# GANtastic3/MaskCycleGAN-VC

Measured on AMD Instinct MI355X. Metric: train iters/s (full G+D step), 80x64 mel bs=1, higher is better.
Workload: dtype f32

## Files before the change

include/mcvc.h:

```cpp
#ifndef MCVC_H
#define MCVC_H

#ifdef __cplusplus
extern "C" {
#endif

#define MCVC_ABI_VERSION 3
#define MCVC_GEN_NPARAMS 110
#define MCVC_DISC_NPARAMS 20
#define MCVC_N_MEL 80

int mcvc_version(void);

int mcvc_set_deterministic(int on);
int mcvc_get_deterministic(void);
int mcvc_set_precise(int on);
int mcvc_get_precise(void);
int mcvc_set_trunk_persistent(int on);

int mcvc_twin_begin(void);
int mcvc_twin_switch(void);
int mcvc_twin_end(void);
int mcvc_twin_launches(void);

long long mcvc_gen_packed_floats(void);
long long mcvc_disc_packed_floats(void);
long long mcvc_gen_stash_floats(int B, int T);
long long mcvc_gen_scratch_floats(int B, int T);
long long mcvc_disc_stash_floats(int B, int T);
// ... 151 lines not shown
int mcvc_instnorm_act_backward(const float* x, const float* gamma, const float* beta, const float* gamma_gate,
                               const float* beta_gate, const float* stats, float* dy, float* dx,
                               float* dgamma, float* dbeta, float* dgamma_gate, float* dbeta_gate,
                               int N, int C, int H, int W, int act, void* stream);

int mcvc_trunk_layer_forward(const float* x, const float* w, const float* bias, const float* gamma, const float* beta, const float* w_gate,
                             const float* bias_gate, const float* gamma_gate, const float* beta_gate, const float* residual, float* conv_out,
                             float* stats, float* y, int B, int Cin, int T4, int Cout, int KW, void* stream);

int mcvc_batched_gemm(const float* a, const float* b, float* c, int nbatch, int M, int N, int K, int lda, int ldb, int ldc,
                      long long a_stride, long long b_stride, long long c_stride, void* stream);

int mcvc_bias_grad(const float* dy, float* db, int N, int C, int P, void* stream);
int mcvc_act_forward(float* x, float* y, int N, int C, int P, int act, void* stream);
int mcvc_act_backward(const float* x, float* dy, float* dx, int N, int C, int P, int act, void* stream);
int mcvc_fif_input(const float* x, const float* mask, float* xin, int N, int P, void* stream);
int mcvc_fif_input_grad(const float* dxin, const float* mask, float* dx, int N, int P, int accumulate, void* stream);

int mcvc_trace_enable(int on);
int mcvc_trace_kinds(void);
const char* mcvc_trace_kind_name(int kind);
int mcvc_trace_collect(double* out);
int mcvc_trace_collect_raw(double* out, int max_records);

#ifdef __cplusplus
}
#endif
#endif
```

maskcyclegan-vc_amd/csrc/fewout_kernels.hip:

```cpp
#include "mcvc_common.h"
#include "trace.h"
#include "launch.h"
#include <stdlib.h>

namespace {

constexpr int kFewTW = 64;
constexpr int kFewTH = 16;
constexpr int kFewCC = 4;

__device__ __attribute__((aligned(16))) float g_few_zero[64];

__device__ __forceinline__ void glds4(const float* g, float* l)
{
    __builtin_amdgcn_global_load_lds((const __attribute__((address_space(1))) void*)g,
                                     (__attribute__((address_space(3))) void*)l, 4, 0, 0);
}

struct FewArgs {
    const float* x; const float* w; const float* bias;
    float* y; float* y_slabs;
    long long x_sb, x_sc, y_sb, y_sc, slab_stride;
    int x_sh, y_sh, y_sw;
    int Cin, H, W, Cout, OH, OW, KH, pad_h, pad_w;
// ... 537 lines not shown
            }
        }
    }
    __syncthreads();
    if (rg < ngr) red[rg * ntap + tap] = acc;
    __syncthreads();
    if (tid < ntap && (int)blockIdx.y < units) {
        float s = 0.f;
        for (int g = 0; g < ngr; ++g) s += red[g * ntap + tid];
        float* d = a.dw + (long long)ci * ntap + tid;
        if (gridDim.y > 1) unsafeAtomicAdd(d, s); else *d += s;
    }
}

constexpr int kCin1Band = 20;
struct WgradCin1KArgs { const float* x; long long x_sn; int x_sh; const float* dy; long long dy_sn; long long dy_sc; int dy_sh; float* dw; int NB; int H; int W; };
__global__ void __launch_bounds__(256) wgrad_cin1_kernel(const Twin<WgradCin1KArgs> tw)
{
    const WgradCin1KArgs ka_ = tw.v[blockIdx.z];
    const float* __restrict__ x = ka_.x;
    long long x_sn = ka_.x_sn;
    int x_sh = ka_.x_sh;
    const float* __restrict__ dy = ka_.dy;
    long long dy_sn = ka_.dy_sn;
    long long dy_sc = ka_.dy_sc;
    int dy_sh = ka_.dy_sh;
    float* __restrict__ dw = ka_.dw;
    int NB = ka_.NB;
    int H = ka_.H;
    int W = ka_.W;
    extern __shared__ float sm[];
    const int XW = W + 2;
    float* xs = sm;
    float* red = sm + (kCin1Band + 2) * XW;
    const int tid = threadIdx.x, co = blockIdx.x;
    const int bands = (H + kCin1Band - 1) / kCin1Band;
    const int units = NB * bands;
    float acc[9];
#pragma unroll
    for (int t = 0; t < 9; ++t) acc[t] = 0.f;
    for (int u = blockIdx.y; u < units; u += gridDim.y) {
        const int n = u / bands, h0 = (u - n * bands) * kCin1Band;
        const int rows = (H - h0 < kCin1Band) ? H - h0 : kCin1Band;
        const float* xp = x + (long long)n * x_sn;
        __syncthreads();
        for (int i = tid; i < (rows + 2) * XW; i += 256) {
            const int r = i / XW, c = i - r * XW;
            const int ih = h0 + r - 1, iw = c - 1;
            xs[i] = (ih >= 0 && ih < H && iw >= 0 && iw < W) ? xp[(long long)ih * x_sh + iw] : 0.f;
        }
        __syncthreads();
        const float* dp = dy + (long long)n * dy_sn + (long long)co * dy_sc + (long long)h0 * dy_sh;
        for (int i = tid; i < rows * W; i += 256) {
            const int r = i / W, c = i - r * W;
            const float d = dp[(long long)r * dy_sh + c];
            const float* xr = xs + r * XW + c;
#pragma unroll
            for (int kh = 0; kh < 3; ++kh)
#pragma unroll
                for (int kw = 0; kw < 3; ++kw) acc[kh * 3 + kw] = fmaf(d, xr[kh * XW + kw], acc[kh * 3 + kw]);
        }
    }
#pragma unroll
    for (int t = 0; t < 9; ++t) {
#pragma unroll
        for (int o = 32; o > 0; o >>= 1) acc[t] += __shfl_xor(acc[t], o, 64);
    }
    __syncthreads();
    if ((tid & 63) == 0) {
#pragma unroll
        for (int t = 0; t < 9; ++t) red[(tid >> 6) * 9 + t] = acc[t];
    }
    __syncthreads();
    if (tid < 9 && (int)blockIdx.y < units) {
        const float v = (red[tid] + red[9 + tid]) + (red[18 + tid] + red[27 + tid]);
        float* d = dw + co * 9 + tid;
        if (gridDim.y > 1) unsafeAtomicAdd(d, v); else *d += v;
    }
}

}

namespace {

constexpr int kW1Ch = 16, kW1PW = 84;
template <int BAND> constexpr int kW1PlaneOf = (BAND + 4) * kW1PW + 4;
constexpr int kW1DyW = 64 + 32;
struct W1Args {
    const float* x; long long x_sn, x_sc; int x_sh;
    const float* dy; long long dy_sn; int dy_sh;
    float* dw;
// ... 91 lines not shown
    }
}

}

namespace {

constexpr int kW2Co = 64;
template <int BAND> constexpr int kW2DyPitch = BAND * 64 + 4;
constexpr int kW2XP = 84;
struct W2Args {
    const float* x; long long x_sn, x_sc; int x_sh;
    const float* dy; long long dy_sn, dy_sc; int dy_sh;
    float* dw;
    int N, Cin, Cout, H, W, bands, units, atomic;
};
template <int CI, int kW2Band>
__global__ void __launch_bounds__(256, 2) wgrad_cin2_mfma_kernel(const Twin<W2Args> tw)
{
    constexpr int kW2DyP = kW2DyPitch<kW2Band>;
    const W2Args a = tw.v[blockIdx.z];
    extern __shared__ __attribute__((aligned(16))) float sm[];
    float* dys = sm;
    float* xs = sm + kW2Co * kW2DyP;
    const int tid = threadIdx.x, lane = tid & 63;
    const int wave = __builtin_amdgcn_readfirstlane(tid >> 6);
    const int ln = lane & 15, kq = lane >> 4;
    const int co0 = blockIdx.x * kW2Co;
    typedef float f32x4w __attribute__((ext_vector_type(4)));
    f32x4w acc[CI][5];
#pragma unroll
    for (int ci = 0; ci < CI; ++ci)
#pragma unroll
        for (int kh = 0; kh < 5; ++kh) acc[ci][kh] = f32x4w{0.f, 0.f, 0.f, 0.f};
    constexpr int P4 = kW2XP / 4, XR = kW2Band + 4;
    for (int u = blockIdx.y; u < a.units; u += gridDim.y) {
        const int n = u / a.bands, h0 = (u - n * a.bands) * kW2Band;
        __syncthreads();
        {
            constexpr int NIT = kW2Co * kW2Band * 16 / 256;
            float4 v[NIT];
#pragma unroll
            for (int it = 0; it < NIT; ++it) {
                const int i = tid + it * 256;
                const int co = i / (kW2Band * 16), rem = i - co * (kW2Band * 16);
                const int r = rem >> 4, c4 = rem & 15;
                v[it] = make_float4(0.f, 0.f, 0.f, 0.f);
                if (co0 + co < a.Cout && h0 + r < a.H)
                    v[it] = *reinterpret_cast<const float4*>(a.dy + (long long)n * a.dy_sn + (long long)(co0 + co) * a.dy_sc + (long long)(h0 + r) * a.dy_sh + 4 * c4);
            }
#pragma unroll
            for (int it = 0; it < NIT; ++it) {
                const int i = tid + it * 256;
// ... 42 lines not shown
    __syncthreads();
    float* red = sm;
    const int per = a.Cin * 75;
#pragma unroll
    for (int ci = 0; ci < CI; ++ci) {
        if (ci >= a.Cin) break;
#pragma unroll
        for (int kh = 0; kh < 5; ++kh)
#pragma unroll
            for (int q = 0; q < 4; ++q) {
                const int kw = 4 * kq + q;
                if (kw < 15) red[(wave * 16 + ln) * per + (ci * 5 + kh) * 15 + kw] = acc[ci][kh][q];
            }
    }
    __syncthreads();
    int nco = a.Cout - co0; if (nco > kW2Co) nco = kW2Co;
    float* d0 = a.dw + (long long)co0 * per;
    for (int i = tid; i < nco * per; i += 256) {
        if (a.atomic) unsafeAtomicAdd(d0 + i, red[i]); else d0[i] += red[i];
    }
}

}

bool mcvc_wgrad_cin2_applies(const ConvProblem& p, const WgradIO& io)
{
    static const int en = mcvc_knob("MCVC_WGRAD_CIN2_MFMA", 1);
    return en && p.Cin >= 1 && p.Cin <= 2 && p.KH == 5 && p.KW == 15 && p.stride == 1 && p.pad_h == 2 && p.pad_w == 7 && p.W == 64 && p.OH == p.H &&
           p.OW == p.W && (io.x_sh & 3) == 0 && (io.x_sc & 3) == 0 && (io.x_sb & 3) == 0 && (io.dy_sh & 3) == 0 && (io.dy_sc & 3) == 0 &&
           (io.dy_sb & 3) == 0 && ((reinterpret_cast<unsigned long long>(io.x) | reinterpret_cast<unsigned long long>(io.dy)) & 15ull) == 0;
}

int mcvc_wgrad_cin2_launch(const ConvProblem& p, int NB, const WgradIO& io, float* dw, hipStream_t s)
{
// ... 2 lines not shown
    w.x = io.x; w.x_sn = io.x_sb; w.x_sc = io.x_sc; w.x_sh = io.x_sh;
    w.dy = io.dy; w.dy_sn = io.dy_sb; w.dy_sc = io.dy_sc; w.dy_sh = io.dy_sh; w.dw = dw;
    const int blocks = cdiv_i(p.Cout, kW2Co);
    const int band = ((long long)blocks * NB * cdiv_i(p.H, 4) < 256) ? 2 : 4;
    w.N = NB; w.Cin = p.Cin; w.Cout = p.Cout; w.H = p.H; w.W = p.W; w.bands = cdiv_i(p.H, band); w.units = NB * w.bands;
    int nch = 1;
    static const int wgs = mcvc_knob("MCVC_WGRAD_CIN2_WGS", 512);
    if (!mcvc_deterministic())
        while (2 * nch <= w.units && blocks * nch < wgs) nch *= 2;
    w.atomic = nch > 1 ? 1 : 0;
    size_t lds = (size_t)(kW2Co * (band * 64 + 4) + 2 * (band + 4) * kW2XP) * sizeof(float);
    const size_t lds_out = (size_t)kW2Co * p.Cin * 75 * sizeof(float);
    if (lds < lds_out) lds = lds_out;
    TraceScope ts(K_WGRAD_4x1, s, 2.0 * NB * p.H * p.W * p.Cout * p.Cin * p.KH * p.KW, 4.0 * ((double)NB * p.Cout * p.H * p.W + (double)NB * p.Cin * p.H * p.W));
    const dim3 grid((unsigned)blocks, (unsigned)nch);
    if (p.Cin == 1) { if (band == 2) mcvc_launch((wgrad_cin2_mfma_kernel<1, 2>), grid, dim3(256), lds, s, w); else mcvc_launch((wgrad_cin2_mfma_kernel<1, 4>), grid, dim3(256), lds, s, w); }
    else { if (band == 2) mcvc_launch((wgrad_cin2_mfma_kernel<2, 2>), grid, dim3(256), lds, s, w); else mcvc_launch((wgrad_cin2_mfma_kernel<2, 4>), grid, dim3(256), lds, s, w); }
    return (int)hipGetLastError();
}

bool mcvc_wgrad_cout1_applies(const ConvProblem& p)
{
    if (p.Cout != 1 || p.stride != 1 || p.KH * p.KW > 128 || p.OH != p.H || p.OW != p.W) return false;
    const int XW = p.W + p.KW - 1;
    const size_t lds = ((size_t)(p.H + p.KH - 1) * XW + (size_t)p.H * p.W + 256) * sizeof(float);
    return lds <= 64 * 1024;
}

int mcvc_wgrad_cout1_launch(const ConvProblem& p, int NB, const WgradIO& io, float* dw, hipStream_t s)
{
    if (!mcvc_wgrad_cout1_applies(p)) return MCVC_ERR_INVALID;
    FewWgradArgs a{};
// ... 34 lines not shown

bool mcvc_wgrad_cin1_applies(const ConvProblem& p)
{
    return p.Cin == 1 && p.KH == 3 && p.KW == 3 && p.stride == 1 && p.pad_h == 1 && p.pad_w == 1 && p.OH == p.H && p.OW == p.W && p.W <= 512;
}

int mcvc_wgrad_cin1_launch(const ConvProblem& p, int NB, const WgradIO& io, float* dw, hipStream_t s)
{
    if (!mcvc_wgrad_cin1_applies(p)) return MCVC_ERR_INVALID;
    const int units = NB * cdiv_i(p.H, kCin1Band);
    int nchunk = 1;
    if (!mcvc_deterministic())
        while (2 * nchunk <= units && p.Cout * nchunk < 1024) nchunk *= 2;
    const size_t lds = ((size_t)(kCin1Band + 2) * (p.W + 2) + 36) * sizeof(float);
    TraceScope ts(K_WGRAD_SMALLK, s, 2.0 * NB * p.H * p.W * p.Cout * 9, 4.0 * ((double)NB * p.Cout * p.H * p.W + (double)NB * p.H * p.W));
    mcvc_launch(wgrad_cin1_kernel, dim3((unsigned)p.Cout, (unsigned)nchunk), dim3(256), lds, s, WgradCin1KArgs{io.x, io.x_sb, io.x_sh, io.dy, io.dy_sb, io.dy_sc, io.dy_sh, dw, NB, p.H, p.W});
    return (int)hipGetLastError();
}
```

maskcyclegan-vc_amd/csrc/mcvc_common.h:

```cpp
#pragma once
#include <hip/hip_runtime.h>
#include <stdint.h>
#include <stddef.h>

typedef float f32x16 __attribute__((ext_vector_type(16)));
typedef float f32x4 __attribute__((ext_vector_type(4)));

#define MCVC_OK 0
#define MCVC_ERR_INVALID 1001
#define MCVC_ERR_WORKSPACE 1002

int mcvc_deterministic();

#ifdef MCVC_EXPERIMENTS
#include <cstdlib>
static inline int mcvc_knob(const char* name, int dflt) { const char* e = getenv(name); return e ? atoi(e) : dflt; }
static inline bool mcvc_knob_set(const char* name) { return getenv(name) != nullptr; }
#else
static inline int mcvc_knob(const char*, int dflt) { return dflt; }
static inline bool mcvc_knob_set(const char*) { return false; }
#endif

static inline int cdiv_i(int a, int b) { return (a + b - 1) / b; }
static inline long long cdiv_ll(long long a, long long b) { return (a + b - 1) / b; }
// ... 141 lines not shown
int mcvc_disc_out_fwd_launch(const float* x, const float* w, const float* bias, float* logit, float* out, int NB, int C, int H, int W, hipStream_t s);
int mcvc_disc_conv1_fwd_launch(const float* x, const float* w, const float* bias, float* c0, float* y0, int NB, int Cout, int H, int W, hipStream_t s, int xs = 0);
int mcvc_disc_out_dgrad_launch(const float* dlogit, const float* w, float* dx, int NB, int C, int H, int W, hipStream_t s);

struct WgradIO {
    const float* x; long long x_sb, x_sc; int x_sh;
    const float* dy; long long dy_sb, dy_sc; int dy_sh;
};
int mcvc_wgrad_launch(const ConvProblem& p, int NB, const WgradIO& io, float* dw, float* slabs, long long slab_cap_floats, hipStream_t s);
bool mcvc_wgrad_cin2_applies(const ConvProblem& p, const WgradIO& io);
int mcvc_wgrad_cin2_launch(const ConvProblem& p, int NB, const WgradIO& io, float* dw, hipStream_t s);
bool mcvc_wgrad_cout1_applies(const ConvProblem& p);
bool mcvc_wgrad_cin1_applies(const ConvProblem& p);
int mcvc_wgrad_cin1_launch(const ConvProblem& p, int NB, const WgradIO& io, float* dw, hipStream_t s);
int mcvc_wgrad_cout1_launch(const ConvProblem& p, int NB, const WgradIO& io, float* dw, hipStream_t s);
long long mcvc_wgrad_plan_slab_floats(const ConvProblem& p, int NB);

struct SmallKJob { const float* x; const float* dy; float* dw; int Cin, Cout; int xB; };
#define MCVC_SMALLK_MAX_JOBS 24
int mcvc_wgrad_smallk_batch_launch(const SmallKJob* jobs, int njobs, int B, int T4, hipStream_t s);
bool mcvc_wgrad_smallk_batch_applies(int B, int T4);

int mcvc_norm_fwd_launch(const NormArgs& a, hipStream_t s);
int mcvc_norm_bwd_launch(const NormBwdArgs& a, hipStream_t s);
int mcvc_act_fwd_launch(const ActArgs& a, hipStream_t s);
int mcvc_act_bwd_launch(const ActBwdArgs& a, hipStream_t s);
```

maskcyclegan-vc_amd/csrc/net.hip:

```cpp
#include "mcvc_common.h"
#include "twin.h"
#include "pack.h"
#include "misc.h"
#include "trunk.h"
#include "wino.h"
#include "wino4.h"
#include "sgemm.h"
#include "sampler.h"
#include "audio.h"
#include "vocoder.h"
#include "griffinlim.h"
#include "../../include/mcvc.h"
#include <string.h>
#include <algorithm>
#include <map>
#include <mutex>
#include <vector>

static int g_deterministic = [] { const char* e = getenv("MCVC_DETERMINISTIC"); return (e && atoi(e) != 0) ? 1 : 0; }();
int mcvc_deterministic() { return g_deterministic; }

namespace {

constexpr float kInEps = 1e-5f;

struct View { float* p; long long sb, sc; int sh; };
struct CView { const float* p; long long sb, sc; int sh; };
static inline CView cv(const View& v) { return CView{v.p, v.sb, v.sc, v.sh}; }

struct Exec {
    hipStream_t s;
    bool dry;
    int err;
    bool fine_ms = false;
    float* slabs;
// ... 1619 lines not shown
        CView dyv{GB, 512LL * 20 * W4, 20LL * W4, W4};
        conv_wgrad(ex, g.ds2, G, B, 40, W2, CView{st + o.y2, 256LL * 40 * W2, 40LL * W2, W2}, dyv);
        conv_dgrad(ex, g.ds2, packed, B, 40, W2, dyv, View{GA, 256LL * 40 * W2, 40LL * W2, W2}, (long long)B * 256 * 40 * W2, 0, 1, &ns);
    }
    if (milestones && ex.fine_ms) record_milestone(ex, milestones[2]);
    GB = nextGB();
    norm_bwd(ex, st + o.c2, 512LL * 40 * W2, 40LL * W2, normp(P, G, 6, 7, 10, 11), st + o.s2, GA, 256LL * 40 * W2, 40LL * W2, W2,
             (long long)B * 256 * 40 * W2, ns, GB, 512LL * 40 * W2, 40LL * W2, W2, 0, B, 256, 40, W2, ACT_GLU);
    {
        CView dyv{GB, 512LL * 40 * W2, 40LL * W2, W2};
        conv_wgrad(ex, g.ds1, G, B, 80, T, CView{st + o.y1, 128LL * 80 * T, 80LL * T, T}, dyv);
        conv_dgrad(ex, g.ds1, packed, B, 80, T, dyv, View{GA, 128LL * 80 * T, 80LL * T, T}, (long long)B * 128 * 80 * T, 0, 1, &ns);
    }
    if (milestones && ex.fine_ms) record_milestone(ex, milestones[3]);
    GB = nextGB();
    act_bwd(ex, st + o.c1, GA, (long long)B * 128 * 80 * T, ns, GB, B, 128, 80 * T, ACT_GLU);
    {
        CView dyv{GB, 256LL * 80 * T, 80LL * T, T};
        ex.br1_on_main = (dx == nullptr) ? 1 : 0;
        conv_wgrad(ex, g.conv1, G, B, 80, T, CView{st + o.xin, 2LL * 80 * T, 80LL * T, T}, dyv);
        ex.br1_on_main = 0;
        conv_bias_grad(ex, g.conv1, G, B, dyv, 80 * T);
        if (dx) {
            conv_dgrad(ex, g.conv1, packed, B, 80, T, dyv, View{GA, 2LL * 80 * T, 80LL * T, T}, (long long)B * 2 * 80 * T, 0, 1, &ns);
            if (!ex.dry) ex.fail(mcvc_mask_grad_launch(GA, ex.slabs, (long long)B * 2 * 80 * T, ns, mask, dx, B, 80 * T, 2, accumulate_dx, ex.s));
        }
    }
    if (ex.no_join) ex.readers.clear(); else join_aux(ex);
}

struct DiscNet { ConvSpec conv1, ds[3], outc; long long packed_floats; };
static DiscNet build_disc()
{
    DiscNet n{};
    long long cur = 0;
    n.conv1 = mk(1, 128, 1, 3, 3, 1, 1, 1, 0, 1, -1, -1, 1);
    n.ds[0] = mk(128, 256, 1, 3, 3, 2, 1, 1, 2, 3, -1, -1, 0);
// ... 147 lines not shown
                     GB, (long long)Co * pl, pl, pitch, 0, B, Co, Ho, Wo, ACT_SILU);
            ex.wgrad_x_xs = 1;
            conv_wgrad(ex, n.ds[i], G, B, Hi, Wi, CView{hin, (long long)Ci * 4 * xpl, 4 * xpl, Wi}, CView{GB, (long long)Co * pl, pl, pitch});
            ex.wgrad_x_xs = 0;
            conv_dgrad_igemm(ex, n.ds[i], packed, B, Hi, Wi, GB, View{GA, (long long)Ci * Hi * Wi, (long long)Hi * Wi, Wi}, (long long)B * Ci * Hi * Wi, 0, 1, &ns);
            continue;
        }
        norm_bwd(ex, st + o.c[i], (long long)Co * Ho * Wo, (long long)Ho * Wo, normp(P, G, 4 + 4 * i, 5 + 4 * i), st + o.s[i],
                 GA, (long long)Co * Ho * Wo, (long long)Ho * Wo, Wo, (long long)B * Co * Ho * Wo, ns,
                 GB, (long long)Co * Ho * Wo, (long long)Ho * Wo, Wo, 0, B, Co, Ho, Wo, ACT_SILU);
        CView dyv{GB, (long long)Co * Ho * Wo, (long long)Ho * Wo, Wo};
        conv_wgrad(ex, n.ds[i], G, B, Hi, Wi, CView{hin, (long long)Ci * Hi * Wi, (long long)Hi * Wi, Wi}, dyv);
        conv_dgrad(ex, n.ds[i], packed, B, Hi, Wi, dyv, View{GA, (long long)Ci * Hi * Wi, (long long)Hi * Wi, Wi}, (long long)B * Ci * Hi * Wi, 0, 1, &ns);
    }
    GB = nextGB();
    act_bwd(ex, st + o.c0, GA, (long long)B * 128 * 80 * T, ns, GB, B, 128, 80 * T, ACT_SILU);
    {
        CView dyv{GB, 128LL * 80 * T, 80LL * T, T};
        conv_wgrad(ex, n.conv1, G, B, 80, T, CView{st + o.total, 80LL * T, 80LL * T, T}, dyv);
        conv_bias_grad(ex, n.conv1, G, B, dyv, 80 * T);
        if (dx) {
            conv_dgrad(ex, n.conv1, packed, B, 80, T, dyv, View{GA, 80LL * T, 80LL * T, T}, (long long)B * 80 * T, 0, 1, &ns);
            if (!ex.dry) ex.fail(mcvc_mask_grad_launch(GA, ex.slabs, (long long)B * 80 * T, ns, nullptr, dx, B, 80 * T, 1, accumulate_dx, ex.s));
        }
    }
    join_aux(ex);
}

struct Needs { long long slab, wslab, sg, sgw; };

template <class F>
static Needs cached_needs(int kind, int B, int T, F&& dry_run)
// ... 73 lines not shown
int mcvc_twin_end(void)
{
    if (!g_mcvc_twin) return MCVC_ERR_INVALID;
    TwinCtx* t = g_mcvc_twin;
    g_mcvc_twin = nullptr;
    const int phase = t->phase;
    t->phase = 0;
    if (t->err) return t->err;
    if (phase != 2 || t->next != t->recs.size()) return MCVC_ERR_INVALID;
    return 0;
}
int mcvc_twin_launches(void) { return (int)t_twin_ctx.recs.size(); }

int mcvc_set_deterministic(int on) { const int was = g_deterministic; g_deterministic = on ? 1 : 0; return was; }
int mcvc_get_deterministic(void) { return g_deterministic; }
int mcvc_set_precise(int on) { const int was = g_precise; g_precise = on ? 1 : 0; return was; }
int mcvc_get_precise(void) { return g_precise; }
int mcvc_set_trunk_persistent(int on) { const int was = g_trunk_net; g_trunk_net = (on == 2) ? 2 : (on ? 1 : 0); return was; }

long long mcvc_gen_packed_floats(void) { return gen_net().packed_floats; }
long long mcvc_disc_packed_floats(void) { return disc_net().packed_floats; }
int mcvc_gen_out_frames(int T) { return gen_dims(1, T).Wu2; }
int mcvc_disc_out_frames(int T) { return disc_dims(1, T).W[3]; }

long long mcvc_gen_stash_floats(int B, int T) { return gen_stash(gen_dims(B, T)).total; }

long long mcvc_gen_scratch_floats(int B, int T)
{
    const Needs nd = gen_needs(B, T);
    return gen_scratch(gen_dims(B, T)).slabs + nd.slab + nd.sg + nd.sgw + nd.wslab + 64;
// ... 805 lines not shown

int mcvc_act_forward(float* x, float* y, int N, int C, int P, int act, void* stream)
{
    Exec ex{}; ex.s = (hipStream_t)stream;
    act_fwd(ex, x, 0, 1, y, N, C, P, act);
    return ex.err;
}

int mcvc_act_backward(const float* x, float* dy, float* dx, int N, int C, int P, int act, void* stream)
{
    Exec ex{}; ex.s = (hipStream_t)stream;
    act_bwd(ex, x, dy, 0, 1, dx, N, C, P, act);
    return ex.err;
}

int mcvc_fif_input(const float* x, const float* mask, float* xin, int N, int P, void* stream)
{
    return mcvc_prep_input_launch(x, mask, xin, N, P, (hipStream_t)stream);
}

int mcvc_fif_input_grad(const float* dxin, const float* mask, float* dx, int N, int P, int accumulate, void* stream)
{
    return mcvc_mask_grad_launch(dxin, nullptr, 0, 1, mask, dx, N, P, 2, accumulate, (hipStream_t)stream);
}

}
```

maskcyclegan-vc_amd/mask_cyclegan_vc/_hip.py:

```python
from __future__ import annotations

import ctypes
import os
from ctypes import c_float, c_int, c_longlong, c_void_p

import torch

_HERE = os.path.dirname(os.path.abspath(__file__))
LIB_PATH = os.environ.get("MCVC_LIB") or os.path.join(os.path.dirname(_HERE), "lib", "libmcvc_hip.so")

ABI_VERSION = 3
GEN_NPARAMS = 110
DISC_NPARAMS = 20
N_MEL = 80

_lib = None

_PP = ctypes.POINTER(c_void_p)

_SIGS = {
    "mcvc_version": (c_int, []),
    "mcvc_set_deterministic": (c_int, [c_int]),
    "mcvc_get_deterministic": (c_int, []),
    "mcvc_set_precise": (c_int, [c_int]),
    "mcvc_get_precise": (c_int, []),
    "mcvc_set_trunk_persistent": (c_int, [c_int]),
    "mcvc_twin_begin": (c_int, []),
    "mcvc_twin_switch": (c_int, []),
    "mcvc_twin_end": (c_int, []),
    "mcvc_twin_launches": (c_int, []),
    "mcvc_gen_packed_floats": (c_longlong, []),
    "mcvc_disc_packed_floats": (c_longlong, []),
    "mcvc_gen_stash_floats": (c_longlong, [c_int, c_int]),
    "mcvc_gen_scratch_floats": (c_longlong, [c_int, c_int]),
    "mcvc_disc_stash_floats": (c_longlong, [c_int, c_int]),
    "mcvc_disc_scratch_floats": (c_longlong, [c_int, c_int]),
    "mcvc_gen_out_frames": (c_int, [c_int]),
    "mcvc_disc_out_frames": (c_int, [c_int]),
# ... 73 lines not shown
    "mcvc_conv2d_dgrad": (c_int, [c_void_p] * 5 + [c_int] * 11 + [c_void_p]),
    "mcvc_conv2d_wgrad_slab_floats": (c_longlong, [c_int] * 10),
    "mcvc_conv2d_wgrad": (c_int, [c_void_p] * 4 + [c_longlong] + [c_int] * 10 + [c_void_p]),
    "mcvc_layer_packed_floats": (c_longlong, [c_int] * 8),
    "mcvc_layer_scratch_floats": (c_longlong, [c_int] * 11),
    "mcvc_layer_pack": (c_int, [c_void_p] * 5 + [c_int] * 8 + [c_void_p]),
    "mcvc_layer_forward": (c_int, [c_void_p] * 6 + [c_longlong] + [c_int] * 13 + [c_void_p]),
    "mcvc_layer_dgrad": (c_int, [c_void_p] * 6 + [c_longlong] + [c_int] * 12 + [c_void_p]),
    "mcvc_layer_wgrad": (c_int, [c_void_p] * 5 + [c_longlong] + [c_int] * 12 + [c_void_p]),
    "mcvc_trunk_layer_backward": (c_int, [c_void_p] * 19 + [c_int] * 5 + [c_void_p]),
    "mcvc_instnorm_act_forward": (c_int, [c_void_p] * 8 + [c_int] * 5 + [c_void_p]),
    "mcvc_instnorm_act_backward": (c_int, [c_void_p] * 12 + [c_int] * 5 + [c_void_p]),
    "mcvc_trunk_layer_forward": (c_int, [c_void_p] * 13 + [c_int] * 5 + [c_void_p]),
    "mcvc_batched_gemm": (c_int, [c_void_p] * 3 + [c_int] * 7 + [c_longlong] * 3 + [c_void_p]),
    "mcvc_bias_grad": (c_int, [c_void_p, c_void_p, c_int, c_int, c_int, c_void_p]),
    "mcvc_act_forward": (c_int, [c_void_p, c_void_p, c_int, c_int, c_int, c_int, c_void_p]),
    "mcvc_act_backward": (c_int, [c_void_p, c_void_p, c_void_p, c_int, c_int, c_int, c_int, c_void_p]),
    "mcvc_fif_input": (c_int, [c_void_p, c_void_p, c_void_p, c_int, c_int, c_void_p]),
    "mcvc_fif_input_grad": (c_int, [c_void_p, c_void_p, c_void_p, c_int, c_int, c_int, c_void_p]),
    "mcvc_trace_enable": (c_int, [c_int]),
    "mcvc_trace_kinds": (c_int, []),
    "mcvc_trace_kind_name": (ctypes.c_char_p, [c_int]),
    "mcvc_trace_collect": (c_int, [ctypes.POINTER(ctypes.c_double)]),
    "mcvc_trace_collect_raw": (c_int, [ctypes.POINTER(ctypes.c_double), c_int]),
}

EXPORTED_SYMBOLS = tuple(_SIGS)


def lib():
# ... 63 lines not shown
```

Baseline: 177.9.

## Fuse activation backward and bias grad into first-layer weight-gradient kernels

Folds the GLU backward (generator conv1) and SiLU backward (discriminator conv1) into the weight-gradient kernels. Each kernel now sums the split-K gradient slabs, applies the activation derivative, and accumulates the bias gradient while staging dy. This removes separate act_bwd and bias_grad launches and the round trip of the intermediate dy through memory. When dx is needed the generator path can still write dy_out or run the plain wgrad on a side stream. In exchange the wgrad kernels carry more loads and sigmoid math, and the stream and event handling gets more complex.

After: 179.3, median of 3. About the same (+0.8%).

```diff
diff --git a/include/mcvc.h b/include/mcvc.h
--- a/include/mcvc.h
+++ b/include/mcvc.h
@@ -13,6 +13,7 @@
 int mcvc_version(void);
 
 int mcvc_set_deterministic(int on);
+int mcvc_set_first_layer_fusion(int mode);
 int mcvc_get_deterministic(void);
 int mcvc_set_precise(int on);
 int mcvc_get_precise(void);
@@ -194,6 +195,10 @@
 int mcvc_bias_grad(const float* dy, float* db, int N, int C, int P, void* stream);
 int mcvc_act_forward(float* x, float* y, int N, int C, int P, int act, void* stream);
 int mcvc_act_backward(const float* x, float* dy, float* dx, int N, int C, int P, int act, void* stream);
+int mcvc_gen_conv1_backward(const float* xin, const float* g, const float* g_slabs, int nslab, const float* c1, float* dy_out, float* dw,
+                            float* dw_gate, float* db, float* db_gate, int N, int C, int H, int W, void* stream);
+int mcvc_disc_conv1_backward(const float* x, const float* g, const float* g_slabs, int nslab, const float* c0, float* dw, float* db,
+                             int N, int C, int H, int W, void* stream);
 int mcvc_fif_input(const float* x, const float* mask, float* xin, int N, int P, void* stream);
 int mcvc_fif_input_grad(const float* dxin, const float* mask, float* dx, int N, int P, int accumulate, void* stream);
 
diff --git a/maskcyclegan-vc_amd/csrc/fewout_kernels.hip b/maskcyclegan-vc_amd/csrc/fewout_kernels.hip
--- a/maskcyclegan-vc_amd/csrc/fewout_kernels.hip
+++ b/maskcyclegan-vc_amd/csrc/fewout_kernels.hip
@@ -575,7 +575,12 @@
 }
 
 constexpr int kCin1Band = 20;
-struct WgradCin1KArgs { const float* x; long long x_sn; int x_sh; const float* dy; long long dy_sn; long long dy_sc; int dy_sh; float* dw; int NB; int H; int W; };
+__device__ __forceinline__ float fl_sigmoid(float v) { return 1.0f / (1.0f + expf(-v)); }
+struct WgradCin1KArgs {
+    const float* x; long long x_sn; int x_sh; const float* dy; long long dy_sn; long long dy_sc; int dy_sh; float* dw; int NB; int H; int W;
+    const float* slabs; long long slab_stride; int nslab; const float* c0; long long c_sn; float* db;
+};
+template <bool ACT>
 __global__ void __launch_bounds__(256) wgrad_cin1_kernel(const Twin<WgradCin1KArgs> tw)
 {
     const WgradCin1KArgs ka_ = tw.v[blockIdx.z];
@@ -595,6 +600,7 @@
     float* xs = sm;
     float* red = sm + (kCin1Band + 2) * XW;
     const int tid = threadIdx.x, co = blockIdx.x;
+    float bsum = 0.f;
     const int bands = (H + kCin1Band - 1) / kCin1Band;
     const int units = NB * bands;
     float acc[9];
@@ -614,7 +620,21 @@
         const float* dp = dy + (long long)n * dy_sn + (long long)co * dy_sc + (long long)h0 * dy_sh;
         for (int i = tid; i < rows * W; i += 256) {
             const int r = i / W, c = i - r * W;
-            const float d = dp[(long long)r * dy_sh + c];
+            float d = dp[(long long)r * dy_sh + c];
+            if (ACT) {
+                const long long go = (long long)n * dy_sn + (long long)co * dy_sc + (long long)(h0 + r) * dy_sh + c;
+                for (int sl = 1; sl < ka_.nslab; sl += 4) {
+                    float u[4];
+#pragma unroll
+                    for (int k = 0; k < 4; ++k) { const int s_ = (sl + k < ka_.nslab) ? sl + k : ka_.nslab - 1; u[k] = ka_.slabs[(long long)(s_ - 1) * ka_.slab_stride + go]; }
+#pragma unroll
+                    for (int k = 0; k < 4; ++k) if (sl + k < ka_.nslab) d += u[k];
+                }
+                const float x0 = ka_.c0[(long long)n * ka_.c_sn + (long long)co * dy_sc + (long long)(h0 + r) * dy_sh + c];
+                const float sg = fl_sigmoid(x0);
+                d = d * (sg * (1.0f + x0 * (1.0f - sg)));
+                bsum += d;
+            }
             const float* xr = xs + r * XW + c;
 #pragma unroll
             for (int kh = 0; kh < 3; ++kh)
@@ -626,16 +646,26 @@
     for (int t = 0; t < 9; ++t) {
 #pragma unroll
         for (int o = 32; o > 0; o >>= 1) acc[t] += __shfl_xor(acc[t], o, 64);
+    }
+    if (ACT) {
+#pragma unroll
+        for (int o = 32; o > 0; o >>= 1) bsum += __shfl_xor(bsum, o, 64);
     }
     __syncthreads();
     if ((tid & 63) == 0) {
 #pragma unroll
         for (int t = 0; t < 9; ++t) red[(tid >> 6) * 9 + t] = acc[t];
+        if (ACT) red[36 + (tid >> 6)] = bsum;
     }
     __syncthreads();
     if (tid < 9 && (int)blockIdx.y < units) {
         const float v = (red[tid] + red[9 + tid]) + (red[18 + tid] + red[27 + tid]);
         float* d = dw + co * 9 + tid;
+        if (gridDim.y > 1) unsafeAtomicAdd(d, v); else *d += v;
+    }
+    if (ACT && tid == 9 && (int)blockIdx.y < units && ka_.db) {
+        const float v = (red[36] + red[37]) + (red[38] + red[39]);
+        float* d = ka_.db + co;
         if (gridDim.y > 1) unsafeAtomicAdd(d, v); else *d += v;
     }
 }
@@ -757,8 +787,23 @@
     const float* dy; long long dy_sn, dy_sc; int dy_sh;
     float* dw;
     int N, Cin, Cout, H, W, bands, units, atomic;
+    const float* g; const float* slabs; long long slab_stride; int nslab; const float* c; long long c_sn;
+    float* dy_out; float* dw1; float* db[2];
 };
-template <int CI, int kW2Band>
+__device__ __forceinline__ float4 w2_ld4(const float* p) { return *reinterpret_cast<const float4*>(p); }
+__device__ __forceinline__ float4 w2_add4(const float4& a, const float4& b) { return make_float4(a.x + b.x, a.y + b.y, a.z + b.z, a.w + b.w); }
+__device__ __forceinline__ float4 w2_slab_sum4(float4 t, const float* slabs, long long stride, long long off, int nslab)
+{
+    for (int sl = 1; sl < nslab; sl += 4) {
+        float4 u[4];
+#pragma unroll
+        for (int k = 0; k < 4; ++k) { const int s_ = (sl + k < nslab) ? sl + k : nslab - 1; u[k] = w2_ld4(slabs + (long long)(s_ - 1) * stride + off); }
+#pragma unroll
+        for (int k = 0; k < 4; ++k) if (sl + k < nslab) t = w2_add4(t, u[k]);
+    }
+    return t;
+}
+template <int CI, int kW2Band, bool GLU>
 __global__ void __launch_bounds__(256, 2) wgrad_cin2_mfma_kernel(const Twin<W2Args> tw)
 {
     constexpr int kW2DyP = kW2DyPitch<kW2Band>;
@@ -777,9 +822,76 @@
 #pragma unroll
         for (int kh = 0; kh < 5; ++kh) acc[ci][kh] = f32x4w{0.f, 0.f, 0.f, 0.f};
     constexpr int P4 = kW2XP / 4, XR = kW2Band + 4;
+    constexpr int kStageIt = kW2Co * kW2Band * 16 / 256;
+    const int br = (GLU && co0 >= a.Cout) ? 1 : 0;
+    const int cb0 = co0 - br * a.Cout;
+    float bacc[GLU ? kStageIt : 1];
+#pragma unroll
+    for (int it = 0; it < (GLU ? kStageIt : 1); ++it) bacc[it] = 0.f;
     for (int u = blockIdx.y; u < a.units; u += gridDim.y) {
         const int n = u / a.bands, h0 = (u - n * a.bands) * kW2Band;
         __syncthreads();
+        if constexpr (GLU) {
+            constexpr int LPC = kW2Band * 16, CS = 256 / LPC;
+            constexpr int CH = kW2Band == 2 ? 4 : 2;
+            const int co_t = tid / LPC, r = (tid % LPC) >> 4, c4 = tid & 15;
+            const long long P = (long long)a.H * 64;
+            const bool ok = h0 + r < a.H;
+            const long long po = (long long)(h0 + r) * 64 + 4 * c4;
+            const long long go = ((long long)n * a.Cout + cb0 + co_t) * P + po;
+            const float* cp = a.c + (long long)n * a.c_sn + (long long)(cb0 + co_t) * P + po;
+            const float* dp = a.dy + (long long)n * a.dy_sn + (long long)(co0 + co_t) * a.dy_sc + (long long)(h0 + r) * a.dy_sh + 4 * c4;
+            float* op = a.dy_out + ((long long)n * 2 * a.Cout + co0 + co_t) * P + po;
+            float* lp = dys + co_t * kW2DyP + r * 64 + 4 * c4;
+#pragma unroll
+            for (int base = 0; base < kStageIt; base += CH) {
+                float4 gv[CH], vv[CH], tv[CH], sv[CH][4];
+#pragma unroll
+                for (int k = 0; k < CH; ++k) {
+                    const long long cs = (long long)(base + k) * CS;
+                    gv[k] = vv[k] = tv[k] = make_float4(0.f, 0.f, 0.f, 0.f);
+                    if (ok) {
+                        if (a.g) {
+                            gv[k] = w2_ld4(a.g + go + cs * P);
+                            vv[k] = w2_ld4(cp + cs * P); tv[k] = w2_ld4(cp + (cs + a.Cout) * P);
+                            if (a.nslab > 1) {
+#pragma unroll
+                                for (int q = 0; q < 4; ++q) {
+                                    const int s_ = (1 + q < a.nslab) ? 1 + q : a.nslab - 1;
+                                    sv[k][q] = w2_ld4(a.slabs + (long long)(s_ - 1) * a.slab_stride + go + cs * P);
+                                }
+                            }
+                        } else {
+                            gv[k] = w2_ld4(dp + cs * a.dy_sc);
+                        }
+                    }
+                }
+#pragma unroll
+                for (int k = 0; k < CH; ++k) {
+                    const long long cs = (long long)(base + k) * CS;
+                    float4 d = gv[k];
+                    if (a.g && ok) {
+                        if (a.nslab > 1) {
+#pragma unroll
+                            for (int q = 0; q < 4; ++q) if (1 + q < a.nslab) d = w2_add4(d, sv[k][q]);
+                            if (a.nslab > 5) d = w2_slab_sum4(d, a.slabs + 4 * a.slab_stride, a.slab_stride, go + cs * P, a.nslab - 4);
+                        }
+                        const float dv[4] = {d.x, d.y, d.z, d.w}, xv[4] = {vv[k].x, vv[k].y, vv[k].z, vv[k].w}, tg[4] = {tv[k].x, tv[k].y, tv[k].z, tv[k].w};
+                        float o[4];
+#pragma unroll
+                        for (int e = 0; e < 4; ++e) {
+                            const float sg = fl_sigmoid(tg[e]);
+                            o[e] = br ? dv[e] * xv[e] * sg * (1.0f - sg) : dv[e] * sg;
+                        }
+                        d = make_float4(o[0], o[1], o[2], o[3]);
+                        if (a.dy_out) *reinterpret_cast<float4*>(op + cs * P) = d;
+                    }
+                    *reinterpret_cast<float4*>(lp + (base + k) * CS * kW2DyP) = d;
+                    bacc[base + k] += (d.x + d.y) + (d.z + d.w);
+                }
+                __builtin_amdgcn_sched_barrier(0);
+            }
+        } else
         {
             constexpr int NIT = kW2Co * kW2Band * 16 / 256;
             float4 v[NIT];
@@ -852,10 +964,24 @@
             }
     }
     __syncthreads();
-    int nco = a.Cout - co0; if (nco > kW2Co) nco = kW2Co;
-    float* d0 = a.dw + (long long)co0 * per;
+    int nco = a.Cout - cb0; if (nco > kW2Co) nco = kW2Co;
+    float* d0 = (br ? a.dw1 : a.dw) + (long long)cb0 * per;
     for (int i = tid; i < nco * per; i += 256) {
         if (a.atomic) unsafeAtomicAdd(d0 + i, red[i]); else d0[i] += red[i];
+    }
+    if constexpr (GLU) {
+        constexpr int LPC = kW2Band * 16;
+        float* db = a.db[br];
+#pragma unroll
+        for (int it = 0; it < kStageIt; ++it) {
+            float v = bacc[it];
+#pragma unroll
+            for (int o = LPC / 2; o > 0; o >>= 1) v += __shfl_xor(v, o, 64);
+            if (db && (tid & (LPC - 1)) == 0) {
+                float* d = db + cb0 + (tid + it * 256) / LPC;
+                if (a.atomic) unsafeAtomicAdd(d, v); else *d += v;
+            }
+        }
     }
 }
 
@@ -888,8 +1014,40 @@
     if (lds < lds_out) lds = lds_out;
     TraceScope ts(K_WGRAD_4x1, s, 2.0 * NB * p.H * p.W * p.Cout * p.Cin * p.KH * p.KW, 4.0 * ((double)NB * p.Cout * p.H * p.W + (double)NB * p.Cin * p.H * p.W));
     const dim3 grid((unsigned)blocks, (unsigned)nch);
-    if (p.Cin == 1) { if (band == 2) mcvc_launch((wgrad_cin2_mfma_kernel<1, 2>), grid, dim3(256), lds, s, w); else mcvc_launch((wgrad_cin2_mfma_kernel<1, 4>), grid, dim3(256), lds, s, w); }
-    else { if (band == 2) mcvc_launch((wgrad_cin2_mfma_kernel<2, 2>), grid, dim3(256), lds, s, w); else mcvc_launch((wgrad_cin2_mfma_kernel<2, 4>), grid, dim3(256), lds, s, w); }
+    if (p.Cin == 1) { if (band == 2) mcvc_launch((wgrad_cin2_mfma_kernel<1, 2, false>), grid, dim3(256), lds, s, w); else mcvc_launch((wgrad_cin2_mfma_kernel<1, 4, false>), grid, dim3(256), lds, s, w); }
+    else { if (band == 2) mcvc_launch((wgrad_cin2_mfma_kernel<2, 2, false>), grid, dim3(256), lds, s, w); else mcvc_launch((wgrad_cin2_mfma_kernel<2, 4, false>), grid, dim3(256), lds, s, w); }
+    return (int)hipGetLastError();
+}
+
+int mcvc_wgrad_cin2_glu_launch(const ConvProblem& p, int NB, const WgradIO& io, const ActGradSrc* g, float* dy_out, float* dw0, float* dw1,
+                               float* db0, float* db1, hipStream_t s)
+{
+    if (!mcvc_wgrad_cin2_applies(p, io) || (p.Cout % kW2Co) != 0 || !dw0 || !dw1) return MCVC_ERR_INVALID;
+    W2Args w{};
+    w.x = io.x; w.x_sn = io.x_sb; w.x_sc = io.x_sc; w.x_sh = io.x_sh;
+    w.dy = io.dy; w.dy_sn = io.dy_sb; w.dy_sc = io.dy_sc; w.dy_sh = io.dy_sh; w.dw = dw0; w.dw1 = dw1; w.db[0] = db0; w.db[1] = db1;
+    if (g) {
+        if (!g->g || !g->c || g->nslab < 1 || (g->nslab > 1 && (!g->slabs || (g->slab_stride & 3))) || (g->c_sb & 3)) return MCVC_ERR_INVALID;
+        if ((reinterpret_cast<unsigned long long>(g->g) | reinterpret_cast<unsigned long long>(g->c) | reinterpret_cast<unsigned long long>(g->slabs) |
+             reinterpret_cast<unsigned long long>(dy_out)) & 15ull) return MCVC_ERR_INVALID;
+        w.g = g->g; w.slabs = g->slabs; w.slab_stride = g->slab_stride; w.nslab = g->nslab; w.c = g->c; w.c_sn = g->c_sb; w.dy_out = dy_out;
+    } else if (!io.dy) return MCVC_ERR_INVALID;
+    const int blocks = p.Cout / kW2Co;
+    const int band = ((long long)blocks * NB * cdiv_i(p.H, 4) < 256) ? 2 : 4;
+    w.N = NB; w.Cin = p.Cin; w.Cout = p.Cout; w.H = p.H; w.W = p.W; w.bands = cdiv_i(p.H, band); w.units = NB * w.bands;
+    int nch = 1;
+    static const int wgs = mcvc_knob("MCVC_WGRAD_CIN2_WGS", 512);
+    if (!mcvc_deterministic())
+        while (2 * nch <= w.units && blocks * nch < wgs) nch *= 2;
+    w.atomic = nch > 1 ? 1 : 0;
+    size_t lds = (size_t)(kW2Co * (band * 64 + 4) + 2 * (band + 4) * kW2XP) * sizeof(float);
+    const size_t lds_out = (size_t)kW2Co * p.Cin * 75 * sizeof(float);
+    if (lds < lds_out) lds = lds_out;
+    TraceScope ts(K_WGRAD_4x1, s, 2.0 * NB * p.H * p.W * 2 * p.Cout * p.Cin * p.KH * p.KW,
+                  4.0 * ((double)NB * 2 * p.Cout * p.H * p.W * (g ? 1.0 + 0.5 * g->nslab + (dy_out ? 1 : 0) : 1.0) + (double)NB * p.Cin * p.H * p.W));
+    const dim3 grid((unsigned)(2 * blocks), (unsigned)nch);
+    if (band == 2) mcvc_launch((wgrad_cin2_mfma_kernel<2, 2, true>), grid, dim3(256), lds, s, w);
+    else mcvc_launch((wgrad_cin2_mfma_kernel<2, 4, true>), grid, dim3(256), lds, s, w);
     return (int)hipGetLastError();
 }
 
@@ -954,6 +1112,22 @@
         while (2 * nchunk <= units && p.Cout * nchunk < 1024) nchunk *= 2;
     const size_t lds = ((size_t)(kCin1Band + 2) * (p.W + 2) + 36) * sizeof(float);
     TraceScope ts(K_WGRAD_SMALLK, s, 2.0 * NB * p.H * p.W * p.Cout * 9, 4.0 * ((double)NB * p.Cout * p.H * p.W + (double)NB * p.H * p.W));
-    mcvc_launch(wgrad_cin1_kernel, dim3((unsigned)p.Cout, (unsigned)nchunk), dim3(256), lds, s, WgradCin1KArgs{io.x, io.x_sb, io.x_sh, io.dy, io.dy_sb, io.dy_sc, io.dy_sh, dw, NB, p.H, p.W});
+    mcvc_launch(wgrad_cin1_kernel<false>, dim3((unsigned)p.Cout, (unsigned)nchunk), dim3(256), lds, s,
+                WgradCin1KArgs{io.x, io.x_sb, io.x_sh, io.dy, io.dy_sb, io.dy_sc, io.dy_sh, dw, NB, p.H, p.W, nullptr, 0, 1, nullptr, 0, nullptr});
     return (int)hipGetLastError();
 }
+
+int mcvc_wgrad_cin1_silu_launch(const ConvProblem& p, int NB, const float* x, long long x_sb, int x_sh, const ActGradSrc& g, float* dw, float* db, hipStream_t s)
+{
+    if (!mcvc_wgrad_cin1_applies(p) || !x || !g.g || !g.c || !dw || g.nslab < 1 || (g.nslab > 1 && !g.slabs)) return MCVC_ERR_INVALID;
+    const int units = NB * cdiv_i(p.H, kCin1Band);
+    int nchunk = 1;
+    if (!mcvc_deterministic())
+        while (2 * nchunk <= units && p.Cout * nchunk < 1024) nchunk *= 2;
+    const size_t lds = ((size_t)(kCin1Band + 2) * (p.W + 2) + 40) * sizeof(float);
+    const long long P = (long long)p.H * p.W;
+    TraceScope ts(K_WGRAD_SMALLK, s, 2.0 * NB * p.H * p.W * p.Cout * 10, 4.0 * ((double)(g.nslab + 1) * NB * p.Cout * p.H * p.W + (double)NB * p.H * p.W));
+    mcvc_launch(wgrad_cin1_kernel<true>, dim3((unsigned)p.Cout, (unsigned)nchunk), dim3(256), lds, s,
+                WgradCin1KArgs{x, x_sb, x_sh, g.g, (long long)p.Cout * P, P, p.W, dw, NB, p.H, p.W, g.slabs, g.slab_stride, g.nslab, g.c, g.c_sb, db});
+    return (int)hipGetLastError();
+}
diff --git a/maskcyclegan-vc_amd/csrc/mcvc_common.h b/maskcyclegan-vc_amd/csrc/mcvc_common.h
--- a/maskcyclegan-vc_amd/csrc/mcvc_common.h
+++ b/maskcyclegan-vc_amd/csrc/mcvc_common.h
@@ -179,6 +179,10 @@
 bool mcvc_wgrad_cin1_applies(const ConvProblem& p);
 int mcvc_wgrad_cin1_launch(const ConvProblem& p, int NB, const WgradIO& io, float* dw, hipStream_t s);
 int mcvc_wgrad_cout1_launch(const ConvProblem& p, int NB, const WgradIO& io, float* dw, hipStream_t s);
+struct ActGradSrc { const float* g; const float* slabs; long long slab_stride; int nslab; const float* c; long long c_sb; };
+int mcvc_wgrad_cin2_glu_launch(const ConvProblem& p, int NB, const WgradIO& io, const ActGradSrc* g, float* dy_out, float* dw0, float* dw1,
+                               float* db0, float* db1, hipStream_t s);
+int mcvc_wgrad_cin1_silu_launch(const ConvProblem& p, int NB, const float* x, long long x_sb, int x_sh, const ActGradSrc& g, float* dw, float* db, hipStream_t s);
 long long mcvc_wgrad_plan_slab_floats(const ConvProblem& p, int NB);
 
 struct SmallKJob { const float* x; const float* dy; float* dw; int Cin, Cout; int xB; };
diff --git a/maskcyclegan-vc_amd/csrc/net.hip b/maskcyclegan-vc_amd/csrc/net.hip
--- a/maskcyclegan-vc_amd/csrc/net.hip
+++ b/maskcyclegan-vc_amd/csrc/net.hip
@@ -19,6 +19,7 @@
 
 static int g_deterministic = [] { const char* e = getenv("MCVC_DETERMINISTIC"); return (e && atoi(e) != 0) ? 1 : 0; }();
 int mcvc_deterministic() { return g_deterministic; }
+static int g_first_layer = mcvc_knob("MCVC_FIRST_LAYER_FUSION", 1);
 
 namespace {
 
@@ -1668,13 +1669,39 @@
     }
     if (milestones && ex.fine_ms) record_milestone(ex, milestones[3]);
     GB = nextGB();
-    act_bwd(ex, st + o.c1, GA, (long long)B * 128 * 80 * T, ns, GB, B, 128, 80 * T, ACT_GLU);
+    const ConvProblem p1{2, 80, T, 128, 80, T, 5, 15, 1, 2, 7};
+    const WgradIO io1{st + o.xin, 2LL * 80 * T, 80LL * T, T, GB, 256LL * 80 * T, 80LL * T, T};
+    const bool fuse1 = g_first_layer && !ex.dry && G && G[g.conv1.wi[0]] && G[g.conv1.wi[1]] && mcvc_wgrad_cin2_applies(p1, io1);
+    const bool form1 = fuse1 && (dx == nullptr || g_first_layer == 2);
+    if (!form1) act_bwd(ex, st + o.c1, GA, (long long)B * 128 * 80 * T, ns, GB, B, 128, 80 * T, ACT_GLU);
     {
         CView dyv{GB, 256LL * 80 * T, 80LL * T, T};
-        ex.br1_on_main = (dx == nullptr) ? 1 : 0;
-        conv_wgrad(ex, g.conv1, G, B, 80, T, CView{st + o.xin, 2LL * 80 * T, 80LL * T, T}, dyv);
-        ex.br1_on_main = 0;
-        conv_bias_grad(ex, g.conv1, G, B, dyv, 80 * T);
+        float* const db0 = (fuse1 && g.conv1.has_bias_grad) ? G[g.conv1.bi[0]] : nullptr;
+        float* const db1 = (fuse1 && g.conv1.has_bias_grad) ? G[g.conv1.bi[1]] : nullptr;
+        if (form1) {
+            const ActGradSrc src{GA, ex.slabs, (long long)B * 128 * 80 * T, ns, st + o.c1, 256LL * 80 * T};
+            if (dx) wait_readers(ex, GB);
+            ex.fail(mcvc_wgrad_cin2_glu_launch(p1, B, io1, &src, dx ? GB : nullptr, G[g.conv1.wi[0]], G[g.conv1.wi[1]], db0, db1, ex.s));
+        } else if (fuse1) {
+            hipStream_t ws = ex.s;
+            if (ex.s2) {
+                hipEvent_t e = pool_event();
+                ex.fail(mcvc_event_record(e, ex.s));
+                ex.fail(mcvc_stream_wait(ex.s2, e));
+                ws = ex.s2;
+            }
+            ex.fail(mcvc_wgrad_cin2_glu_launch(p1, B, io1, nullptr, nullptr, G[g.conv1.wi[0]], G[g.conv1.wi[1]], db0, db1, ws));
+            if (ex.s2) {
+                hipEvent_t e = pool_event();
+                ex.fail(mcvc_event_record(e, ex.s2));
+                ex.readers.emplace_back((const void*)GB, e);
+            }
+        } else {
+            ex.br1_on_main = (dx == nullptr) ? 1 : 0;
+            conv_wgrad(ex, g.conv1, G, B, 80, T, CView{st + o.xin, 2LL * 80 * T, 80LL * T, T}, dyv);
+            ex.br1_on_main = 0;
+            conv_bias_grad(ex, g.conv1, G, B, dyv, 80 * T);
+        }
         if (dx) {
             conv_dgrad(ex, g.conv1, packed, B, 80, T, dyv, View{GA, 2LL * 80 * T, 80LL * T, T}, (long long)B * 2 * 80 * T, 0, 1, &ns);
             if (!ex.dry) ex.fail(mcvc_mask_grad_launch(GA, ex.slabs, (long long)B * 2 * 80 * T, ns, mask, dx, B, 80 * T, 2, accumulate_dx, ex.s));
@@ -1852,8 +1879,13 @@
         conv_dgrad(ex, n.ds[i], packed, B, Hi, Wi, dyv, View{GA, (long long)Ci * Hi * Wi, (long long)Hi * Wi, Wi}, (long long)B * Ci * Hi * Wi, 0, 1, &ns);
     }
     GB = nextGB();
-    act_bwd(ex, st + o.c0, GA, (long long)B * 128 * 80 * T, ns, GB, B, 128, 80 * T, ACT_SILU);
-    {
+    const ConvProblem p0{1, 80, T, 128, 80, T, 3, 3, 1, 1, 1};
+    const bool fuse0 = g_first_layer && !ex.dry && G && G[n.conv1.wi[0]] && !dx && mcvc_wgrad_cin1_applies(p0) && wgrad_cin1_enabled();
+    if (fuse0) {
+        const ActGradSrc src{GA, ex.slabs, (long long)B * 128 * 80 * T, ns, st + o.c0, 128LL * 80 * T};
+        ex.fail(mcvc_wgrad_cin1_silu_launch(p0, B, st + o.total, 80LL * T, T, src, G[n.conv1.wi[0]], n.conv1.has_bias_grad ? G[n.conv1.bi[0]] : nullptr, ex.s));
+    } else {
+        act_bwd(ex, st + o.c0, GA, (long long)B * 128 * 80 * T, ns, GB, B, 128, 80 * T, ACT_SILU);
         CView dyv{GB, 128LL * 80 * T, 80LL * T, T};
         conv_wgrad(ex, n.conv1, G, B, 80, T, CView{st + o.total, 80LL * T, 80LL * T, T}, dyv);
         conv_bias_grad(ex, n.conv1, G, B, dyv, 80 * T);
@@ -1957,6 +1989,7 @@
 
 int mcvc_set_deterministic(int on) { const int was = g_deterministic; g_deterministic = on ? 1 : 0; return was; }
 int mcvc_get_deterministic(void) { return g_deterministic; }
+int mcvc_set_first_layer_fusion(int mode) { const int was = g_first_layer; g_first_layer = (mode == 2) ? 2 : (mode ? 1 : 0); return was; }
 int mcvc_set_precise(int on) { const int was = g_precise; g_precise = on ? 1 : 0; return was; }
 int mcvc_get_precise(void) { return g_precise; }
 int mcvc_set_trunk_persistent(int on) { const int was = g_trunk_net; g_trunk_net = (on == 2) ? 2 : (on ? 1 : 0); return was; }
@@ -2792,6 +2825,25 @@
     return ex.err;
 }
 
+int mcvc_gen_conv1_backward(const float* xin, const float* g, const float* g_slabs, int nslab, const float* c1, float* dy_out, float* dw,
+                            float* dw_gate, float* db, float* db_gate, int N, int C, int H, int W, void* stream)
+{
+    const ConvProblem p{2, H, W, C, H, W, 5, 15, 1, 2, 7};
+    const long long P = (long long)H * W;
+    const WgradIO io{xin, 2 * P, P, W, nullptr, 2 * C * P, P, W};
+    const ActGradSrc src{g, g_slabs, (long long)N * C * P, nslab, c1, 2 * C * P};
+    return mcvc_wgrad_cin2_glu_launch(p, N, io, &src, dy_out, dw, dw_gate, db, db_gate, (hipStream_t)stream);
+}
+
+int mcvc_disc_conv1_backward(const float* x, const float* g, const float* g_slabs, int nslab, const float* c0, float* dw, float* db,
+                             int N, int C, int H, int W, void* stream)
+{
+    const ConvProblem p{1, H, W, C, H, W, 3, 3, 1, 1, 1};
+    const long long P = (long long)H * W;
+    const ActGradSrc src{g, g_slabs, (long long)N * C * P, nslab, c0, C * P};
+    return mcvc_wgrad_cin1_silu_launch(p, N, x, P, W, src, dw, db, (hipStream_t)stream);
+}
+
 int mcvc_fif_input(const float* x, const float* mask, float* xin, int N, int P, void* stream)
 {
     return mcvc_prep_input_launch(x, mask, xin, N, P, (hipStream_t)stream);
diff --git a/maskcyclegan-vc_amd/mask_cyclegan_vc/_hip.py b/maskcyclegan-vc_amd/mask_cyclegan_vc/_hip.py
--- a/maskcyclegan-vc_amd/mask_cyclegan_vc/_hip.py
+++ b/maskcyclegan-vc_amd/mask_cyclegan_vc/_hip.py
@@ -22,6 +22,7 @@
     "mcvc_version": (c_int, []),
     "mcvc_set_deterministic": (c_int, [c_int]),
     "mcvc_get_deterministic": (c_int, []),
+    "mcvc_set_first_layer_fusion": (c_int, [c_int]),
     "mcvc_set_precise": (c_int, [c_int]),
     "mcvc_get_precise": (c_int, []),
     "mcvc_set_trunk_persistent": (c_int, [c_int]),
@@ -125,6 +126,8 @@
     "mcvc_trunk_layer_forward": (c_int, [c_void_p] * 13 + [c_int] * 5 + [c_void_p]),
     "mcvc_batched_gemm": (c_int, [c_void_p] * 3 + [c_int] * 7 + [c_longlong] * 3 + [c_void_p]),
     "mcvc_bias_grad": (c_int, [c_void_p, c_void_p, c_int, c_int, c_int, c_void_p]),
+    "mcvc_gen_conv1_backward": (c_int, [c_void_p, c_void_p, c_void_p, c_int, c_void_p, c_void_p, c_void_p, c_void_p, c_void_p, c_void_p, c_int, c_int, c_int, c_int, c_void_p]),
+    "mcvc_disc_conv1_backward": (c_int, [c_void_p, c_void_p, c_void_p, c_int, c_void_p, c_void_p, c_void_p, c_int, c_int, c_int, c_int, c_void_p]),
     "mcvc_act_forward": (c_int, [c_void_p, c_void_p, c_int, c_int, c_int, c_int, c_void_p]),
     "mcvc_act_backward": (c_int, [c_void_p, c_void_p, c_void_p, c_int, c_int, c_int, c_int, c_void_p]),
     "mcvc_fif_input": (c_int, [c_void_p, c_void_p, c_void_p, c_int, c_int, c_void_p]),
```
